# YifanXu74/MQ-Det

Hardware: NVIDIA H100
Metric: images/sec MQ-GLIP-T 800x1333, 5 vis-queries, 80-class prompt (higher is better)
Workload: dtype f16

## Files before the change

mqdet_b200/csrc/biattn.cu:

```cuda
#include "common.cuh"
#include "wgmma.cuh"
#include "../../include/mqdet_b200.h"

namespace mqdet {

constexpr int BM = 64;
constexpr int BK = 64;
constexpr int KB_BYTES = 64 * BK * 2;

template <int R>
__device__ __forceinline__ void acc_to_a(const float (&e)[R], int kk, uint32_t (&a)[4]) {
  a[0] = pack_half2(e[8 * kk + 0], e[8 * kk + 1]);
  a[1] = pack_half2(e[8 * kk + 2], e[8 * kk + 3]);
  a[2] = pack_half2(e[8 * kk + 4], e[8 * kk + 5]);
  a[3] = pack_half2(e[8 * kk + 6], e[8 * kk + 7]);
}
__device__ __forceinline__ float quad_max(float v) {
  v = fmaxf(v, __shfl_xor_sync(0xffffffffu, v, 1));
  return fmaxf(v, __shfl_xor_sync(0xffffffffu, v, 2));
}
__device__ __forceinline__ float quad_sum(float v) {
  v += __shfl_xor_sync(0xffffffffu, v, 1);
  return v + __shfl_xor_sync(0xffffffffu, v, 2);
}

constexpr int BT_STEP = 64;
struct BtCfg {
  static constexpr int KT_BYTES = 4 * KB_BYTES;
  static constexpr int Q_BYTES = 4 * KB_BYTES;
  static constexpr int V_BYTES = 256 * BT_STEP * 2;
  static constexpr int STAGE_BYTES = Q_BYTES + V_BYTES;
  static constexpr int SMEM_BYTES = KT_BYTES + 2 * STAGE_BYTES + 1024  + 256 ;
};
static_assert(BtCfg::SMEM_BYTES <= 232448, "biattn_text: dynamic shared memory above the 227 KB per-CTA limit");
struct BtP {
  const float* stat;
  float clamp;
  int nb1, T, N, n_steps;
  int k_bc1, k_bc2, q_bc1, q_bc2, v_bc1, v_bc2;
  const float* rowbias;
  int rb_ld;
  __half* out;
  long o_ld, o_b1, o_b2;
};

template <bool VN>
__global__ void __launch_bounds__(128, 1) biattn_text_kernel(const __grid_constant__ CUtensorMap tma_k,
                                                             const __grid_constant__ CUtensorMap tma_q,
                                                             const __grid_constant__ CUtensorMap tma_v, const BtP p) {
  extern __shared__ uint8_t smem_raw[];
  uint8_t* smem = reinterpret_cast<uint8_t*>((reinterpret_cast<uintptr_t>(smem_raw) + 1023) & ~uintptr_t(1023));
  uint8_t* kt = smem;
  uint8_t* ring = kt + BtCfg::KT_BYTES;
  uint64_t* bars = reinterpret_cast<uint64_t*>(ring + 2 * BtCfg::STAGE_BYTES);
  uint64_t* kt_full = bars;
  uint64_t* full = bars + 1;

  const int tid = threadIdx.x;
  const int mt = blockIdx.x, z = blockIdx.y;
  const int z1 = z % p.nb1, z2 = z / p.nb1;
  const int NS = p.n_steps;
  const int qz1 = p.q_bc1 ? 0 : z1, qz2 = p.q_bc2 ? 0 : z2, vz1 = p.v_bc1 ? 0 : z1, vz2 = p.v_bc2 ? 0 : z2;

  auto issue = [&](int i) {
    uint8_t* st = ring + (i & 1) * BtCfg::STAGE_BYTES;
    uint64_t* bar = &full[i & 1];
    mbar_expect_tx(bar, BtCfg::STAGE_BYTES);
    for (int kb = 0; kb < 4; ++kb) tma_load_4d(st + kb * KB_BYTES, &tma_q, bar, kb * BK, i * BT_STEP, qz1, qz2);
    if (VN)
      for (int cb = 0; cb < 4; ++cb) tma_load_4d(st + BtCfg::Q_BYTES + cb * KB_BYTES, &tma_v, bar, cb * BK, i * BT_STEP, vz1, vz2);
    else
      tma_load_4d(st + BtCfg::Q_BYTES, &tma_v, bar, i * BT_STEP, 0, vz1, vz2);
  };
  if (tid == 0) {
    tma_prefetch_desc(&tma_k);
    tma_prefetch_desc(&tma_q);
    tma_prefetch_desc(&tma_v);
    mbar_init(kt_full, 1);
    mbar_init(&full[0], 1);
    mbar_init(&full[1], 1);
    fence_mbar_init();
    mbar_expect_tx(kt_full, BtCfg::KT_BYTES);
    for (int kb = 0; kb < 4; ++kb)
      tma_load_4d(kt + kb * KB_BYTES, &tma_k, kt_full, kb * BK, mt * BM, p.k_bc1 ? 0 : z1, p.k_bc2 ? 0 : z2);
    issue(0);
    if (NS > 1) issue(1);
  }
  __syncthreads();

  constexpr float L2E = 1.4426950408889634f;
  float m_l2[2] = {0.f, 0.f}, inv[2] = {0.f, 0.f}, gb[2] = {0.f, 0.f}, lsum[2] = {0.f, 0.f};
#pragma unroll
  for (int h = 0; h < 2; ++h) {
    const int t = mt * BM + wg_row(tid, 2 * h);
    if (t < p.T) {
      if (VN) {
        m_l2[h] = -p.stat[(long)z * p.T + t] * L2E;
        if (p.rowbias) gb[h] = p.rowbias[((long)z * p.T + t) * p.rb_ld];
      } else {
        m_l2[h] = -p.stat[((long)z * 2) * p.T + t] * L2E;
        inv[h] = p.stat[((long)z * 2 + 1) * p.T + t];
      }
    }
  }
  const float clampv = p.clamp > 0.f ? p.clamp : 3.0e38f;
  const uint32_t kt_addr = smem_u32(kt);
  float o[128];
#pragma unroll
  for (int i = 0; i < 128; ++i) o[i] = 0.f;
  mbar_wait(kt_full, 0);
  for (int i = 0; i < NS; ++i) {
    const int s = i & 1;
    mbar_wait(&full[s], (i >> 1) & 1);
    const uint32_t q0 = smem_u32(ring + s * BtCfg::STAGE_BYTES), v0 = q0 + BtCfg::Q_BYTES;
    float sc[32];
#pragma unroll
    for (int j = 0; j < 32; ++j) sc[j] = 0.f;
    wgmma_fence_acc(sc);
    wgmma_fence();
#pragma unroll
    for (int kb = 0; kb < 4; ++kb)
#pragma unroll
      for (int k = 0; k < 4; ++k)
        wgmma_ss_m64n64_kk(sc, wg_desc_k_sw128(kt_addr + kb * KB_BYTES + k * 32), wg_desc_k_sw128(q0 + kb * KB_BYTES + k * 32), 1);
    wgmma_commit();
    wgmma_wait<0>();
    wgmma_fence_acc(sc);
    const int nrem = p.N - i * BT_STEP;
#pragma unroll
    for (int j = 0; j < 32; ++j) {
      const int h = (j >> 1) & 1;
      const float a = fminf(fmaxf(sc[j] + gb[h], -clampv), clampv);
      const float f = VN ? a : __half2float(__float2half_rn(a));
      float e = ex2_approx(fmaf(f, L2E, m_l2[h]));
      if (wg_col(tid, j) >= nrem) e = 0.f;
      if (VN) lsum[h] += e;
      sc[j] = e;
    }
    uint32_t pa[4][4];
#pragma unroll
    for (int kk = 0; kk < 4; ++kk) acc_to_a(sc, kk, pa[kk]);
    wgmma_fence_acc(o);
    wgmma_fence();
#pragma unroll
    for (int kk = 0; kk < 4; ++kk) {
      if (VN)
        wgmma_rs_m64n256_kmn(o, pa[kk], wg_desc_mn_sw128(v0 + kk * 2048, KB_BYTES, 1024), 1);
      else
        wgmma_rs_m64n256_kk(o, pa[kk], wg_desc_k_sw128(v0 + kk * 32), 1);
    }
    wgmma_commit();
    wgmma_wait<0>();
    wgmma_fence_acc(o);
    __syncthreads();
    if (tid == 0 && i + 2 < NS) issue(i + 2);
  }
  if (VN) {
#pragma unroll
    for (int h = 0; h < 2; ++h) {
      const float tot = quad_sum(lsum[h]);
      inv[h] = tot > 0.f ? 1.f / tot : 0.f;
    }
  }
  __half* out = p.out + z1 * p.o_b1 + z2 * p.o_b2;
#pragma unroll
  for (int j = 0; j < 128; j += 2) {
    const int h = (j >> 1) & 1;
    const int t = mt * BM + wg_row(tid, j);
    if (t < p.T)
      *reinterpret_cast<__half2*>(out + (long)t * p.o_ld + wg_col(tid, j)) = __floats2half2_rn(o[j] * inv[h], o[j + 1] * inv[h]);
  }
}

struct BiCfg {
  static constexpr int VN_BYTES = 4 * KB_BYTES;
  static constexpr int STAGE_BYTES = 256 * BK * 2;
  static constexpr int MAX_HEADS = 8;
  static constexpr int D_BYTES = 128 * 128 * 4;
  static constexpr int EXTRA_BYTES = (4 * 256 + MAX_HEADS * 256) * 4;
  static constexpr int SMEM_BYTES = VN_BYTES + 2 * STAGE_BYTES + D_BYTES + EXTRA_BYTES + 1024  + 256 ;
};
static_assert(BiCfg::SMEM_BYTES <= 232448, "biattn_image: dynamic shared memory above the 227 KB per-CTA limit");
struct BiP {
  const float* mask;
  const float* bias;
  const float* gamma;
  const __half* res;
  long res_ld, res_b;
  __half* out;
  long o_ld, o_b;
  float* colmax_part;
  const float* gbias;
  int gb_ld;
  float clamp;
  int B, H, T, N, tiles_per_img;
};

__global__ void __launch_bounds__(128, 1) biattn_image_kernel(const __grid_constant__ CUtensorMap tma_q,
                                                              const __grid_constant__ CUtensorMap tma_k,
                                                              const __grid_constant__ CUtensorMap tma_m, const BiP p) {
  extern __shared__ uint8_t smem_raw[];
  uint8_t* smem = reinterpret_cast<uint8_t*>((reinterpret_cast<uintptr_t>(smem_raw) + 1023) & ~uintptr_t(1023));
  uint8_t* vnt = smem;
  uint8_t* ring = vnt + BiCfg::VN_BYTES;
  float* dsum = reinterpret_cast<float*>(ring + 2 * BiCfg::STAGE_BYTES);
  float* cmx = dsum + 128 * 128;
  float* gk = cmx + 4 * 256;
  uint64_t* bars = reinterpret_cast<uint64_t*>(gk + BiCfg::MAX_HEADS * 256);
  uint64_t* vn_full = bars;
  uint64_t* full = bars + 1;

  const int tid = threadIdx.x, warp = tid >> 5, lane = tid & 31;
  const int H = p.H;
  const int b = blockIdx.x / p.tiles_per_img, ti = blockIdx.x - b * p.tiles_per_img, m0 = ti * BM;
  const int nq = 8 * H;
  auto issue = [&](int q) {
    const int h = q >> 3, kb = q & 3;
    uint64_t* bar = &full[q & 1];
    mbar_expect_tx(bar, BiCfg::STAGE_BYTES);
    tma_load_4d(ring + (q & 1) * BiCfg::STAGE_BYTES, (q & 4) ? &tma_m : &tma_k, bar, kb * BK, 0, h, b);
  };
  if (tid == 0) {
    tma_prefetch_desc(&tma_q);
    tma_prefetch_desc(&tma_k);
    tma_prefetch_desc(&tma_m);
    mbar_init(vn_full, 1);
    mbar_init(&full[0], 1);
    mbar_init(&full[1], 1);
    fence_mbar_init();
    mbar_expect_tx(vn_full, BiCfg::VN_BYTES);
    for (int kb = 0; kb < 4; ++kb) tma_load_4d(vnt + kb * KB_BYTES, &tma_q, vn_full, kb * BK, m0, b, 0);
    issue(0);
    issue(1);
  }
  constexpr float L2E = 1.4426950408889634f;
  const float NEG_INF = __int_as_float(0xff800000);
  const float clampv = p.clamp > 0.f ? p.clamp : 3.0e38f;
  for (int t = tid; t < 256; t += 128) {
    const bool kept = t < p.T && (!p.mask || p.mask[(long)b * p.T + t] != 0.f);
    for (int hh = 0; hh < H; ++hh)
      gk[hh * 256 + t] = !kept ? NEG_INF : (p.gbias ? p.gbias[(((long)b * H + hh) * p.T + t) * p.gb_ld] : 0.f);
  }
  __syncthreads();
  bool valid[2];
#pragma unroll
  for (int h = 0; h < 2; ++h) valid[h] = m0 + wg_row(tid, 2 * h) < p.N;
  const uint32_t vn_addr = smem_u32(vnt);
  int q = 0;
  auto ring_wait = [&](int qq) { mbar_wait(&full[qq & 1], (qq >> 1) & 1); };
  auto ring_release = [&](int qq) {
    __syncthreads();
    if (tid == 0 && qq + 2 < nq) issue(qq + 2);
  };
  mbar_wait(vn_full, 0);
  for (int h = 0; h < H; ++h) {
    float sc[128];
#pragma unroll
    for (int j = 0; j < 128; ++j) sc[j] = 0.f;
    for (int kb = 0; kb < 4; ++kb, ++q) {
      ring_wait(q);
      const uint32_t b0 = smem_u32(ring + (q & 1) * BiCfg::STAGE_BYTES);
      wgmma_fence_acc(sc);
      wgmma_fence();
#pragma unroll
      for (int k = 0; k < 4; ++k)
        wgmma_ss_m64n256_kk(sc, wg_desc_k_sw128(vn_addr + kb * KB_BYTES + k * 32), wg_desc_k_sw128(b0 + k * 32), 1);
      wgmma_commit();
      wgmma_wait<0>();
      wgmma_fence_acc(sc);
      ring_release(q);
    }
#pragma unroll
    for (int j = 0; j < 128; j += 4) {
#pragma unroll
      for (int c = 0; c < 2; ++c) {
        float m = fmaxf(valid[0] ? sc[j + c] : NEG_INF, valid[1] ? sc[j + 2 + c] : NEG_INF);
        m = fmaxf(m, __shfl_xor_sync(0xffffffffu, m, 4));
        m = fmaxf(m, __shfl_xor_sync(0xffffffffu, m, 8));
        m = fmaxf(m, __shfl_xor_sync(0xffffffffu, m, 16));
        if (lane < 4) cmx[warp * 256 + wg_col(tid, j + c)] = m;
      }
    }
    __syncthreads();
    for (int t = tid; t < p.T; t += 128) {
      float c4 = fmaxf(fmaxf(cmx[t], cmx[256 + t]), fmaxf(cmx[512 + t], cmx[768 + t]));
      if (p.gbias) c4 += p.gbias[(((long)b * H + h) * p.T + t) * p.gb_ld];
      c4 = fminf(fmaxf(c4, -clampv), clampv);
      p.colmax_part[(((long)b * H + h) * p.tiles_per_img + ti) * p.T + t] = c4;
    }
    const float* kl = gk + h * 256;
    float mr[2] = {NEG_INF, NEG_INF};
#pragma unroll
    for (int j = 0; j < 128; ++j) mr[(j >> 1) & 1] = fmaxf(mr[(j >> 1) & 1], sc[j] + kl[wg_col(tid, j)]);
    float ml2[2];
    bool uniform[2];
#pragma unroll
    for (int r = 0; r < 2; ++r) {
      const float m_raw = quad_max(mr[r]);
      uniform[r] = (m_raw == NEG_INF);
      ml2[r] = uniform[r] ? 0.f : fminf(fmaxf(m_raw, -clampv), clampv) * L2E;
    }
    float ls[2] = {0.f, 0.f};
#pragma unroll
    for (int j = 0; j < 128; ++j) {
      const int r = (j >> 1) & 1, c = wg_col(tid, j);
      const float kk = kl[c];
      float ev = (kk == NEG_INF) ? 0.f : ex2_approx(fmaf(fminf(fmaxf(sc[j] + kk, -clampv), clampv), L2E, -ml2[r]));
      if (uniform[r]) ev = (c < p.T) ? 1.f : 0.f;
      sc[j] = ev;
      ls[r] += ev;
    }
    const float inv[2] = {1.f / quad_sum(ls[0]), 1.f / quad_sum(ls[1])};
#pragma unroll
    for (int j = 0; j < 128; ++j) sc[j] *= inv[(j >> 1) & 1];
    uint32_t pa[16][4];
#pragma unroll
    for (int kk = 0; kk < 16; ++kk) acc_to_a(sc, kk, pa[kk]);
    float d[128];
#pragma unroll
    for (int j = 0; j < 128; ++j) d[j] = 0.f;
    for (int kb = 0; kb < 4; ++kb, ++q) {
      ring_wait(q);
      const uint32_t b0 = smem_u32(ring + (q & 1) * BiCfg::STAGE_BYTES);
      wgmma_fence_acc(d);
      wgmma_fence();
#pragma unroll
      for (int k = 0; k < 4; ++k) wgmma_rs_m64n256_kk(d, pa[kb * 4 + k], wg_desc_k_sw128(b0 + k * 32), 1);
      wgmma_commit();
      wgmma_wait<0>();
      wgmma_fence_acc(d);
      ring_release(q);
    }
#pragma unroll
    for (int j = 0; j < 128; ++j) dsum[j * 128 + tid] = (h == 0 ? 0.f : dsum[j * 128 + tid]) + d[j];
  }
#pragma unroll 4
  for (int j = 0; j < 128; j += 2) {
    const long row = m0 + wg_row(tid, j);
    const int c = wg_col(tid, j);
    if (row >= p.N) continue;
    float o0 = dsum[j * 128 + tid], o1 = dsum[(j + 1) * 128 + tid];
    const float g0 = p.gamma ? p.gamma[c] : 1.f, g1 = p.gamma ? p.gamma[c + 1] : 1.f;
    const float b0 = p.bias ? p.bias[c] : 0.f, b1 = p.bias ? p.bias[c + 1] : 0.f;
    o0 = (o0 + b0) * g0;
    o1 = (o1 + b1) * g1;
    if (p.res) {
      const float2 r = __half22float2(*reinterpret_cast<const __half2*>(p.res + (long)b * p.res_b + row * p.res_ld + c));
      o0 += r.x;
      o1 += r.y;
    }
    *reinterpret_cast<__half2*>(p.out + (long)b * p.o_b + row * p.o_ld + c) = __floats2half2_rn(o0, o1);
  }
}

__global__ void colmax_reduce_kernel(const float* __restrict__ part, int tiles, int T, float* __restrict__ out) {
  const int z = blockIdx.x;
  for (int t = threadIdx.x; t < T; t += blockDim.x) {
    float m = __int_as_float(0xff800000);
    const float* src = part + (long)z * tiles * T + t;
    for (int i = 0; i < tiles; ++i) m = fmaxf(m, src[(long)i * T]);
    out[(long)z * T + t] = m;
  }
}

}

using namespace mqdet;

static int text_launch(bool vn, const float* rowbias, int64_t rb_ld, const void* k, int64_t k_ld, int64_t k_b1, int64_t k_b2, const void* q, int64_t q_ld, int64_t q_b1,
                       int64_t q_b2, const void* v, int64_t v_ld, int64_t v_b1, int64_t v_b2, const float* stat, float clamp,
                       void* out, int64_t o_ld, int64_t o_b1, int64_t o_b2, int64_t nb1, int64_t nb2, int64_t T, int64_t N,
                       int64_t Np, int64_t d, void* stream) {
  MQ_REQUIRE(k && q && v && stat && out, "biattn_text: null pointer");
  MQ_REQUIRE(d == 256, "biattn_text: head dim must be 256 (embed 2048 / 8 heads, fuse_helper.py:186-189), got %ld", (long)d);
  MQ_REQUIRE(T >= 1 && T <= 256 && N >= 1 && Np >= N && (Np % 8) == 0, "biattn_text: need 1 <= T <= 256, Np >= N, Np %% 8 == 0");
  MQ_REQUIRE(nb1 >= 1 && nb2 >= 1 && nb1 * nb2 <= 65535, "biattn_text: bad batch");
  const int64_t lds[] = {k_ld, k_b1, k_b2, q_ld, q_b1, q_b2, v_ld, v_b1, v_b2, o_ld, o_b1, o_b2};
  for (int64_t x : lds) MQ_REQUIRE((x % 8) == 0, "biattn_text: strides must be multiples of 8 elements");
  MQ_REQUIRE(((uintptr_t)k % 16) == 0 && ((uintptr_t)q % 16) == 0 && ((uintptr_t)v % 16) == 0 && ((uintptr_t)out % 16) == 0,
             "biattn_text: operands must be 16-byte aligned");
  CUtensorMap mk, mq, mv;
  BtP p;
  memset(&p, 0, sizeof(p));
  int rc = make_operand_map(&mk, k, T, d, k_ld, (int)nb1, k_b1, (int)nb2, k_b2, BM, &p.k_bc1, &p.k_bc2);
  if (rc) return rc;
  rc = make_operand_map(&mq, q, N, d, q_ld, (int)nb1, q_b1, (int)nb2, q_b2, BT_STEP, &p.q_bc1, &p.q_bc2);
  if (rc) return rc;
  if (vn)
    rc = make_operand_map(&mv, v, N, 256, v_ld, (int)nb1, v_b1, (int)nb2, v_b2, BT_STEP, &p.v_bc1, &p.v_bc2);
  else
    rc = make_operand_map(&mv, v, d, Np, v_ld, (int)nb1, v_b1, (int)nb2, v_b2, 256, &p.v_bc1, &p.v_bc2);
  if (rc) return rc;
  MQ_REQUIRE((nb1 == 1 || o_b1 != 0) && (nb2 == 1 || o_b2 != 0), "biattn_text: output batch strides must be non-zero");
  p.out = (__half*)out;
  p.o_ld = o_ld;
  p.o_b1 = o_b1;
  p.o_b2 = o_b2;
  p.stat = stat;
  p.clamp = clamp;
  p.nb1 = (int)nb1;
  p.T = (int)T;
  p.N = (int)N;
  p.n_steps = (int)((N + BT_STEP - 1) / BT_STEP);
  p.rowbias = rowbias;
  p.rb_ld = (int)(rb_ld > 0 ? rb_ld : 1);
  dim3 grid((unsigned)((T + BM - 1) / BM), (unsigned)(nb1 * nb2));
  if (vn) {
    rc = ensure_dyn_smem(reinterpret_cast<const void*>(&biattn_text_kernel<true>), BtCfg::SMEM_BYTES);
    if (rc) return rc;
    biattn_text_kernel<true><<<grid, 128, BtCfg::SMEM_BYTES, (cudaStream_t)stream>>>(mk, mq, mv, p);
  } else {
    rc = ensure_dyn_smem(reinterpret_cast<const void*>(&biattn_text_kernel<false>), BtCfg::SMEM_BYTES);
    if (rc) return rc;
    biattn_text_kernel<false><<<grid, 128, BtCfg::SMEM_BYTES, (cudaStream_t)stream>>>(mk, mq, mv, p);
  }
  return check_launch("biattn_text_kernel");
}

extern "C" int mqdet_biattn_text(const void* k, int64_t k_ld, int64_t k_b1, int64_t k_b2, const void* q, int64_t q_ld,
                                 int64_t q_b1, int64_t q_b2, const void* vvT, int64_t v_ld, int64_t v_b1, int64_t v_b2,
                                 const float* stat, float clamp, void* out, int64_t o_ld, int64_t o_b1, int64_t o_b2,
                                 int64_t nb1, int64_t nb2, int64_t T, int64_t N, int64_t Np, int64_t d, void* stream) {
  return text_launch(false, nullptr, 0, k, k_ld, k_b1, k_b2, q, q_ld, q_b1, q_b2, vvT, v_ld, v_b1, v_b2, stat, clamp, out, o_ld, o_b1, o_b2,
                     nb1, nb2, T, N, Np, d, stream);
}

extern "C" int mqdet_biattn_text_vn(const void* k, int64_t k_ld, int64_t k_b1, int64_t k_b2, const void* q, int64_t q_ld,
                                    int64_t q_b1, int64_t q_b2, const void* vn, int64_t vn_ld, int64_t vn_b1, int64_t vn_b2,
                                    const float* colmax, const float* rowbias, int64_t rb_ld, float clamp, void* out, int64_t o_ld,
                                    int64_t o_b1, int64_t o_b2, int64_t nb1, int64_t nb2, int64_t T, int64_t N, void* stream) {
  return text_launch(true, rowbias, rb_ld, k, k_ld, k_b1, k_b2, q, q_ld, q_b1, q_b2, vn, vn_ld, vn_b1, vn_b2, colmax, clamp, out, o_ld, o_b1,
                     o_b2, nb1, nb2, T, N, (N + 7) / 8 * 8, 256, stream);
}

extern "C" int64_t mqdet_biattn_image_workspace_floats(int64_t B, int64_t H, int64_t N, int64_t T) {
  return B * H * ((N + BM - 1) / BM) * T;
}

extern "C" int mqdet_biattn_image(const void* vn, int64_t vn_ld, int64_t vn_b, const void* gT, int64_t g_ld, int64_t g_bh,
                                  int64_t g_b, const float* gbias, int64_t gb_ld, const void* mT, int64_t m_ld, int64_t m_bh,
                                  int64_t m_b, const float* bias, const float* gamma, const void* res, int64_t res_ld,
                                  int64_t res_b, const float* mask, float clamp, void* out, int64_t o_ld, int64_t o_b,
                                  float* colmax, float* workspace, int64_t B, int64_t H, int64_t N, int64_t T, void* stream) {
  MQ_REQUIRE(vn && gT && mT && out && colmax && workspace, "biattn_image: null pointer");
  MQ_REQUIRE(B >= 1 && H >= 1 && H <= BiCfg::MAX_HEADS && N >= 1 && T >= 8 && T <= 256 && (T % 8) == 0,
             "biattn_image: need B, N >= 1, 1 <= H <= 8, 8 <= T <= 256, T %% 8 == 0 (got B=%ld H=%ld N=%ld T=%ld)", (long)B, (long)H, (long)N, (long)T);
  const int64_t lds[] = {vn_ld, vn_b, g_ld, g_bh, g_b, m_ld, m_bh, m_b, o_ld, o_b, res ? res_ld : 0, res ? res_b : 0};
  for (int64_t x : lds) MQ_REQUIRE((x % 8) == 0, "biattn_image: strides must be multiples of 8 elements");
  MQ_REQUIRE(((uintptr_t)vn % 16) == 0 && ((uintptr_t)gT % 16) == 0 && ((uintptr_t)mT % 16) == 0 && ((uintptr_t)out % 16) == 0 &&
                 ((uintptr_t)res % 16) == 0 && ((uintptr_t)bias % 16) == 0 && ((uintptr_t)gamma % 16) == 0,
             "biattn_image: operands must be 16-byte aligned");
  CUtensorMap mq, mk, mm;
  int bc1, bc2;
  int rc = make_operand_map(&mq, vn, N, 256, vn_ld, (int)B, vn_b, 1, 0, BM, &bc1, &bc2);
  if (rc) return rc;
  MQ_REQUIRE((H == 1 || (g_bh != 0 && m_bh != 0)) && (B == 1 || (g_b != 0 && m_b != 0)), "biattn_image: head / image strides must be non-zero");
  rc = make_operand_map(&mk, gT, T, 256, g_ld, (int)H, g_bh, (int)B, g_b, 256, &bc1, &bc2);
  if (rc) return rc;
  rc = make_operand_map(&mm, mT, 256, T, m_ld, (int)H, m_bh, (int)B, m_b, 256, &bc1, &bc2);
  if (rc) return rc;
  MQ_REQUIRE(B == 1 || o_b != 0, "biattn_image: output batch stride must be non-zero");
  BiP p;
  memset(&p, 0, sizeof(p));
  p.mask = mask;
  p.bias = bias;
  p.gamma = gamma;
  p.res = (const __half*)res;
  p.res_ld = res_ld;
  p.res_b = res_b;
  p.out = (__half*)out;
  p.o_ld = o_ld;
  p.o_b = o_b;
  p.colmax_part = workspace;
  p.gbias = gbias;
  p.gb_ld = (int)(gb_ld > 0 ? gb_ld : 1);
  p.clamp = clamp;
  p.B = (int)B; p.H = (int)H; p.T = (int)T; p.N = (int)N;
  p.tiles_per_img = (int)((N + BM - 1) / BM);
  rc = ensure_dyn_smem(reinterpret_cast<const void*>(&biattn_image_kernel), BiCfg::SMEM_BYTES);
  if (rc) return rc;
  biattn_image_kernel<<<(unsigned)(p.tiles_per_img * B), 128, BiCfg::SMEM_BYTES, (cudaStream_t)stream>>>(mq, mk, mm, p);
  rc = check_launch("biattn_image_kernel");
  if (rc) return rc;
  colmax_reduce_kernel<<<(unsigned)(B * H), 256, 0, (cudaStream_t)stream>>>(workspace, p.tiles_per_img, (int)T, colmax);
  return check_launch("colmax_reduce_kernel");
}
```

mqdet_b200/csrc/common.cuh:

```cuda
#pragma once
#include <cuda.h>
#include <cuda_runtime.h>
#include <cuda_fp16.h>
#include <stdint.h>
#include <stdio.h>
#include <string.h>

#define MQDET_OK 0
#define MQDET_ERR_ARG -1
#define MQDET_ERR_CUDA -2
#define MQDET_ERR_UNSUPPORTED -3

namespace mqdet {

void set_error(const char* fmt, ...);
int check_launch(const char* what);

#define MQ_REQUIRE(cond, ...)                      \
  do {                                             \
    if (!(cond)) {                                 \
      mqdet::set_error(__VA_ARGS__);               \
      return MQDET_ERR_ARG;                        \
    }                                              \
  } while (0)
// ... 80 lines not shown
  d.pw = pw;
  d.ph = ph;
  return d;
}

__device__ __forceinline__ void token_focal_elem(float x, float y, float alpha, float gamma, float& loss, float& dloss) {
  const float p = 1.f / (1.f + expf(-x));
  const float ce = fmaxf(x, 0.f) - x * y + log1pf(expf(-fabsf(x)));
  const float pt = p * y + (1.f - p) * (1.f - y);
  const float om = 1.f - pt;
  const float mod = powf(om, gamma);
  const float at = alpha >= 0.f ? alpha * y + (1.f - alpha) * (1.f - y) : 1.f;
  loss = at * ce * mod;
  const float dmod = (om > 0.f) ? gamma * powf(om, gamma - 1.f) * (-(2.f * y - 1.f) * p * (1.f - p)) : 0.f;
  dloss = at * ((p - y) * mod + ce * dmod);
}

__device__ __forceinline__ void mbar_init(uint64_t* bar, uint32_t count) {
  asm volatile("mbarrier.init.shared::cta.b64 [%0], %1;" ::"r"(smem_u32(bar)), "r"(count));
}
__device__ __forceinline__ void fence_mbar_init() {
  asm volatile("fence.mbarrier_init.release.cluster;" ::: "memory");
}
__device__ __forceinline__ void sts128(uint32_t addr, uint32_t x, uint32_t y, uint32_t z, uint32_t w) {
  asm volatile("st.shared.v4.b32 [%0], {%1, %2, %3, %4};" ::"r"(addr), "r"(x), "r"(y), "r"(z), "r"(w) : "memory");
}
__device__ __forceinline__ float4 lds128f(uint32_t addr) {
  float4 v;
  asm volatile("ld.shared.v4.f32 {%0, %1, %2, %3}, [%4];" : "=f"(v.x), "=f"(v.y), "=f"(v.z), "=f"(v.w) : "r"(addr) : "memory");
  return v;
}
__device__ __forceinline__ float ex2_approx(float x) {
  float y;
  asm("ex2.approx.ftz.f32 %0, %1;" : "=f"(y) : "f"(x));
  return y;
}
__device__ __forceinline__ uint32_t pack_half2(float x, float y) {
  const __half2 h = __floats2half2_rn(x, y);
  return *reinterpret_cast<const uint32_t*>(&h);
}
__device__ __forceinline__ void ffma2(float& d0, float& d1, float a0, float a1, float s, float b0, float b1) {
  d0 = fmaf(a0, s, b0);
  d1 = fmaf(a1, s, b1);
}
__device__ __forceinline__ void ffma2v(float& d0, float& d1, float a0, float a1, float s0, float s1, float b0, float b1) {
  d0 = fmaf(a0, s0, b0);
  d1 = fmaf(a1, s1, b1);
}
__device__ __forceinline__ void fence_proxy_async() {
  asm volatile("fence.proxy.async.shared::cta;" ::: "memory");
}
__device__ __forceinline__ void mbar_expect_tx(uint64_t* bar, uint32_t bytes) {
  asm volatile("mbarrier.arrive.expect_tx.shared::cta.b64 _, [%0], %1;" ::"r"(smem_u32(bar)),
               "r"(bytes)
               : "memory");
}
__device__ __forceinline__ void mbar_arrive(uint64_t* bar) {
  asm volatile("mbarrier.arrive.shared::cta.b64 _, [%0];" ::"r"(smem_u32(bar)) : "memory");
}
__device__ __forceinline__ void mbar_wait(uint64_t* bar, uint32_t parity) {
  uint32_t addr = smem_u32(bar);
  uint32_t done;
  do {
    asm volatile(
        "{\n"
        ".reg .pred p;\n"
        "mbarrier.try_wait.parity.shared::cta.b64 p, [%1], %2;\n"
        "selp.u32 %0, 1, 0, p;\n"
        "}\n"
        : "=r"(done)
        : "r"(addr), "r"(parity)
        : "memory");
  } while (!done);
}

__device__ __forceinline__ void tma_prefetch_desc(const CUtensorMap* m) {
  asm volatile("prefetch.tensormap [%0];" ::"l"(reinterpret_cast<uint64_t>(m)) : "memory");
}
__device__ __forceinline__ void tma_load_4d(void* smem_dst, const CUtensorMap* m, uint64_t* bar,
                                            int c0, int c1, int c2, int c3) {
  asm volatile(
      "cp.async.bulk.tensor.4d.shared::cluster.global.tile.mbarrier::complete_tx::bytes "
// ... 83 lines not shown
```

mqdet_b200/csrc/gemm.cu:

```cuda
#include "common.cuh"
#include "wgmma.cuh"
#include "../../include/mqdet_b200.h"

namespace mqdet {

struct GemmP {
  const __half* A;
  const __half* B;
  long M, N, K, lda, ldb;
  int nb1, nb2;
  long a_b1, a_b2, b_b1, b_b2;
  void* C;
  int c_dtype;
  long ldc, c_b1, c_b2;
  float alpha;
  int scale_after_bias;
  const float* bias;
  int bias_mode;
  long bias_b1, bias_b2;
  int act;
  float clamp;
  const float* gate;
  int gate_mode, gate_tanh;
  const void* R;
// ... 56 lines not shown
  EPI_NONE_F16,
  EPI_BIAS_F16,
  EPI_BIAS_GELU_F16,
  EPI_BIAS_RES_F32,
};

template <int BN, int STAGES, int EPI>
struct WgCfg {
  static constexpr int A_BYTES = BM * BK * 2;
  static constexpr int B_BYTES = BN * BK * 2;
  static constexpr int STAGE_BYTES = A_BYTES + B_BYTES;
  static constexpr int PITCH = BN + 8;
  static constexpr bool OUT_F32 = EPI == EPI_BIAS_RES_F32;
  static constexpr int ES = OUT_F32 ? 4 : 2;
  static constexpr int PASSES = OUT_F32 ? 2 : 1;
  static constexpr int PASS_COLS = BN / PASSES;
  static constexpr int BOX_COLS = 128 / ES;
  static constexpr int BOXES = PASS_COLS / BOX_COLS;
  static constexpr int EPI_BYTES = EPI == EPI_GENERIC ? 64 * PITCH * 4 : BM * BN * 2;
  static constexpr int SMEM_BYTES = STAGES * STAGE_BYTES + 2 * EPI_BYTES + 1024  + 256 ;
  static_assert(EPI_BYTES % 1024 == 0, "swizzled boxes need 1024-byte alignment");
};

__device__ __forceinline__ void named_bar_sync(int id, int n) { asm volatile("bar.sync %0, %1;" ::"r"(id), "r"(n) : "memory"); }
__device__ __forceinline__ void named_bar_arrive(int id, int n) { asm volatile("bar.arrive %0, %1;" ::"r"(id), "r"(n) : "memory"); }
template <int R>
__device__ __forceinline__ void setmaxnreg_dec() { asm volatile("setmaxnreg.dec.sync.aligned.u32 %0;" ::"n"(R)); }
template <int R>
__device__ __forceinline__ void setmaxnreg_inc() { asm volatile("setmaxnreg.inc.sync.aligned.u32 %0;" ::"n"(R)); }
__device__ __forceinline__ void sts32(uint32_t addr, uint32_t x) { asm volatile("st.shared.b32 [%0], %1;" ::"r"(addr), "r"(x) : "memory"); }
__device__ __forceinline__ void sts64f(uint32_t addr, float x, float y) {
  asm volatile("st.shared.v2.f32 [%0], {%1, %2};" ::"r"(addr), "f"(x), "f"(y) : "memory");
}
__device__ __forceinline__ float2 lds64f(uint32_t addr) {
  float2 v;
  asm volatile("ld.shared.v2.f32 {%0, %1}, [%2];" : "=f"(v.x), "=f"(v.y) : "r"(addr) : "memory");
  return v;
}
template <int ES>
__device__ __forceinline__ uint32_t box_addr(uint32_t base, int r, int c) {
  const int byte = c * ES;
  return base + (byte >> 7) * (BM * 128) + r * 128 + ((((byte >> 4) & 7) ^ (r & 7)) << 4) + (byte & 15);
}

struct TileIdx {
  int n_tile, m_tile, z1, z2;
};
__device__ __forceinline__ TileIdx tile_idx(int t, int n_tiles, int m_tiles, int nb1) {
  TileIdx r;
  const int per_z = n_tiles * m_tiles;
  const int z = t / per_z, rem = t - z * per_z;
  r.m_tile = rem / n_tiles;
  r.n_tile = rem - r.m_tile * n_tiles;
// ... 396 lines not shown
```

Measured before the change: 178.6.

## Warp-specialize bi-attention kernels with producer warpgroup and split score/value consumers

Both bi-attention kernels become warp-specialized. One producer warpgroup drives TMA through full/empty mbarrier rings, and consumer warpgroups rebalance registers with setmaxnreg. The text kernel processes two M-tiles per CTA that share the streamed Q/V ring, and it reuses a single buffer when Q and V alias. The image kernel splits softmax scoring and the P·V product across two warpgroups that hand off probabilities through swizzled shared memory, with part of the accumulator spilled to shared memory. The column-max reduction is also parallelized across 8 warps. This aims to overlap loads, softmax and matmul and to cut full-CTA syncs, at the cost of more complex synchronization and fewer CTAs for the text kernel.

```diff
diff --git a/mqdet_b200/csrc/biattn.cu b/mqdet_b200/csrc/biattn.cu
--- a/mqdet_b200/csrc/biattn.cu
+++ b/mqdet_b200/csrc/biattn.cu
@@ -29,14 +29,16 @@
   static constexpr int KT_BYTES = 4 * KB_BYTES;
   static constexpr int Q_BYTES = 4 * KB_BYTES;
   static constexpr int V_BYTES = 256 * BT_STEP * 2;
-  static constexpr int STAGE_BYTES = Q_BYTES + V_BYTES;
-  static constexpr int SMEM_BYTES = KT_BYTES + 2 * STAGE_BYTES + 1024  + 256 ;
+  static constexpr int RING_BYTES = 2 * (Q_BYTES + V_BYTES);
+  static constexpr int MAX_STAGES = RING_BYTES / Q_BYTES;
+  static constexpr int SMEM_BYTES = 2 * KT_BYTES + RING_BYTES + 1024  + 256 ;
 };
 static_assert(BtCfg::SMEM_BYTES <= 232448, "biattn_text: dynamic shared memory above the 227 KB per-CTA limit");
 struct BtP {
   const float* stat;
   float clamp;
   int nb1, T, N, n_steps;
+  int qv_shared;
   int k_bc1, k_bc2, q_bc1, q_bc2, v_bc1, v_bc2;
   const float* rowbias;
   int rb_ld;
@@ -45,48 +47,72 @@
 };
 
 template <bool VN>
-__global__ void __launch_bounds__(128, 1) biattn_text_kernel(const __grid_constant__ CUtensorMap tma_k,
+__global__ void __launch_bounds__(384, 1) biattn_text_kernel(const __grid_constant__ CUtensorMap tma_k,
                                                              const __grid_constant__ CUtensorMap tma_q,
                                                              const __grid_constant__ CUtensorMap tma_v, const BtP p) {
   extern __shared__ uint8_t smem_raw[];
   uint8_t* smem = reinterpret_cast<uint8_t*>((reinterpret_cast<uintptr_t>(smem_raw) + 1023) & ~uintptr_t(1023));
   uint8_t* kt = smem;
-  uint8_t* ring = kt + BtCfg::KT_BYTES;
-  uint64_t* bars = reinterpret_cast<uint64_t*>(ring + 2 * BtCfg::STAGE_BYTES);
+  uint8_t* ring = kt + 2 * BtCfg::KT_BYTES;
+  uint64_t* bars = reinterpret_cast<uint64_t*>(ring + BtCfg::RING_BYTES);
   uint64_t* kt_full = bars;
-  uint64_t* full = bars + 1;
-
-  const int tid = threadIdx.x;
-  const int mt = blockIdx.x, z = blockIdx.y;
+  uint64_t* full = bars + 2;
+  uint64_t* empty = full + BtCfg::MAX_STAGES;
+
+  const int wg = threadIdx.x >> 7, tid = threadIdx.x & 127;
+  const int z = blockIdx.y;
   const int z1 = z % p.nb1, z2 = z / p.nb1;
   const int NS = p.n_steps;
-  const int qz1 = p.q_bc1 ? 0 : z1, qz2 = p.q_bc2 ? 0 : z2, vz1 = p.v_bc1 ? 0 : z1, vz2 = p.v_bc2 ? 0 : z2;
-
-  auto issue = [&](int i) {
-    uint8_t* st = ring + (i & 1) * BtCfg::STAGE_BYTES;
-    uint64_t* bar = &full[i & 1];
-    mbar_expect_tx(bar, BtCfg::STAGE_BYTES);
-    for (int kb = 0; kb < 4; ++kb) tma_load_4d(st + kb * KB_BYTES, &tma_q, bar, kb * BK, i * BT_STEP, qz1, qz2);
-    if (VN)
-      for (int cb = 0; cb < 4; ++cb) tma_load_4d(st + BtCfg::Q_BYTES + cb * KB_BYTES, &tma_v, bar, cb * BK, i * BT_STEP, vz1, vz2);
-    else
-      tma_load_4d(st + BtCfg::Q_BYTES, &tma_v, bar, i * BT_STEP, 0, vz1, vz2);
-  };
-  if (tid == 0) {
+  const int mt0 = 2 * blockIdx.x;
+  const int ncons = min(2, (p.T - mt0 * BM + BM - 1) / BM);
+  const int stage_bytes = p.qv_shared ? BtCfg::Q_BYTES : BtCfg::Q_BYTES + BtCfg::V_BYTES;
+  const int nst = BtCfg::RING_BYTES / stage_bytes;
+
+  if (threadIdx.x == 0) {
     tma_prefetch_desc(&tma_k);
     tma_prefetch_desc(&tma_q);
     tma_prefetch_desc(&tma_v);
-    mbar_init(kt_full, 1);
-    mbar_init(&full[0], 1);
-    mbar_init(&full[1], 1);
+    mbar_init(&kt_full[0], 1);
+    mbar_init(&kt_full[1], 1);
+    for (int s = 0; s < nst; ++s) {
+      mbar_init(&full[s], 1);
+      mbar_init(&empty[s], 128 * ncons);
+    }
     fence_mbar_init();
-    mbar_expect_tx(kt_full, BtCfg::KT_BYTES);
-    for (int kb = 0; kb < 4; ++kb)
-      tma_load_4d(kt + kb * KB_BYTES, &tma_k, kt_full, kb * BK, mt * BM, p.k_bc1 ? 0 : z1, p.k_bc2 ? 0 : z2);
-    issue(0);
-    if (NS > 1) issue(1);
   }
   __syncthreads();
+
+  if (wg == 0) {
+    setmaxnreg_dec<40>();
+    if (tid == 0) {
+      const int qz1 = p.q_bc1 ? 0 : z1, qz2 = p.q_bc2 ? 0 : z2, vz1 = p.v_bc1 ? 0 : z1, vz2 = p.v_bc2 ? 0 : z2;
+      for (int g = 0; g < ncons; ++g) {
+        mbar_expect_tx(&kt_full[g], BtCfg::KT_BYTES);
+        for (int kb = 0; kb < 4; ++kb)
+          tma_load_4d(kt + g * BtCfg::KT_BYTES + kb * KB_BYTES, &tma_k, &kt_full[g], kb * BK, (mt0 + g) * BM, p.k_bc1 ? 0 : z1,
+                      p.k_bc2 ? 0 : z2);
+      }
+      for (int i = 0; i < NS; ++i) {
+        const int s = i % nst;
+        uint8_t* st = ring + s * stage_bytes;
+        mbar_wait(&empty[s], ((i / nst) & 1) ^ 1);
+        mbar_expect_tx(&full[s], stage_bytes);
+        for (int kb = 0; kb < 4; ++kb) tma_load_4d(st + kb * KB_BYTES, &tma_q, &full[s], kb * BK, i * BT_STEP, qz1, qz2);
+        if (!p.qv_shared) {
+          if (VN)
+            for (int cb = 0; cb < 4; ++cb)
+              tma_load_4d(st + BtCfg::Q_BYTES + cb * KB_BYTES, &tma_v, &full[s], cb * BK, i * BT_STEP, vz1, vz2);
+          else
+            tma_load_4d(st + BtCfg::Q_BYTES, &tma_v, &full[s], i * BT_STEP, 0, vz1, vz2);
+        }
+      }
+    }
+    return;
+  }
+  setmaxnreg_inc<232>();
+  const int g = wg - 1;
+  if (g >= ncons) return;
+  const int mt = mt0 + g;
 
   constexpr float L2E = 1.4426950408889634f;
   float m_l2[2] = {0.f, 0.f}, inv[2] = {0.f, 0.f}, gb[2] = {0.f, 0.f}, lsum[2] = {0.f, 0.f};
@@ -104,15 +130,16 @@
     }
   }
   const float clampv = p.clamp > 0.f ? p.clamp : 3.0e38f;
-  const uint32_t kt_addr = smem_u32(kt);
+  const uint32_t kt_addr = smem_u32(kt + g * BtCfg::KT_BYTES);
+  const uint32_t v_off = p.qv_shared ? 0 : BtCfg::Q_BYTES;
   float o[128];
 #pragma unroll
   for (int i = 0; i < 128; ++i) o[i] = 0.f;
-  mbar_wait(kt_full, 0);
+  mbar_wait(&kt_full[g], 0);
   for (int i = 0; i < NS; ++i) {
-    const int s = i & 1;
-    mbar_wait(&full[s], (i >> 1) & 1);
-    const uint32_t q0 = smem_u32(ring + s * BtCfg::STAGE_BYTES), v0 = q0 + BtCfg::Q_BYTES;
+    const int s = i % nst;
+    mbar_wait(&full[s], (i / nst) & 1);
+    const uint32_t q0 = smem_u32(ring + s * stage_bytes), v0 = q0 + v_off;
     float sc[32];
 #pragma unroll
     for (int j = 0; j < 32; ++j) sc[j] = 0.f;
@@ -152,8 +179,7 @@
     wgmma_commit();
     wgmma_wait<0>();
     wgmma_fence_acc(o);
-    __syncthreads();
-    if (tid == 0 && i + 2 < NS) issue(i + 2);
+    mbar_arrive(&empty[s]);
   }
   if (VN) {
 #pragma unroll
@@ -175,10 +201,16 @@
 struct BiCfg {
   static constexpr int VN_BYTES = 4 * KB_BYTES;
   static constexpr int STAGE_BYTES = 256 * BK * 2;
+  static constexpr int STAGES = 2;
+  static constexpr int M_STAGE_BYTES = 64 * BK * 2;
+  static constexpr int M_STAGES = 4;
+  static constexpr int P_BYTES = 4 * KB_BYTES;
   static constexpr int MAX_HEADS = 8;
-  static constexpr int D_BYTES = 128 * 128 * 4;
-  static constexpr int EXTRA_BYTES = (4 * 256 + MAX_HEADS * 256) * 4;
-  static constexpr int SMEM_BYTES = VN_BYTES + 2 * STAGE_BYTES + D_BYTES + EXTRA_BYTES + 1024  + 256 ;
+  static constexpr int EXTRA_BYTES = (2 * 4 * 256 + MAX_HEADS * 256) * 4;
+  static constexpr int D_REG = 64;
+  static constexpr int D3_BYTES = (128 - D_REG) * 128 * 4;
+  static constexpr int SMEM_BYTES =
+      VN_BYTES + P_BYTES + STAGES * STAGE_BYTES + M_STAGES * M_STAGE_BYTES + EXTRA_BYTES + D3_BYTES + 1024  + 256 ;
 };
 static_assert(BiCfg::SMEM_BYTES <= 232448, "biattn_image: dynamic shared memory above the 227 KB per-CTA limit");
 struct BiP {
@@ -196,150 +228,209 @@
   int B, H, T, N, tiles_per_img;
 };
 
-__global__ void __launch_bounds__(128, 1) biattn_image_kernel(const __grid_constant__ CUtensorMap tma_q,
+__device__ __forceinline__ uint32_t sw128_off(int r, int c) {
+  return (c >> 6) * KB_BYTES + r * 128 + ((((c & 63) >> 3) ^ (r & 7)) << 4) + ((c & 7) << 1);
+}
+
+__global__ void __launch_bounds__(384, 1) biattn_image_kernel(const __grid_constant__ CUtensorMap tma_q,
                                                               const __grid_constant__ CUtensorMap tma_k,
                                                               const __grid_constant__ CUtensorMap tma_m, const BiP p) {
+  constexpr int S = BiCfg::STAGES, MS = BiCfg::M_STAGES;
   extern __shared__ uint8_t smem_raw[];
   uint8_t* smem = reinterpret_cast<uint8_t*>((reinterpret_cast<uintptr_t>(smem_raw) + 1023) & ~uintptr_t(1023));
   uint8_t* vnt = smem;
-  uint8_t* ring = vnt + BiCfg::VN_BYTES;
-  float* dsum = reinterpret_cast<float*>(ring + 2 * BiCfg::STAGE_BYTES);
-  float* cmx = dsum + 128 * 128;
-  float* gk = cmx + 4 * 256;
-  uint64_t* bars = reinterpret_cast<uint64_t*>(gk + BiCfg::MAX_HEADS * 256);
+  uint8_t* pt = vnt + BiCfg::VN_BYTES;
+  uint8_t* ring_g = pt + BiCfg::P_BYTES;
+  uint8_t* ring_m = ring_g + S * BiCfg::STAGE_BYTES;
+  float* cmx = reinterpret_cast<float*>(ring_m + MS * BiCfg::M_STAGE_BYTES);
+  float* gk = cmx + 2 * 4 * 256;
+  float* d3 = gk + BiCfg::MAX_HEADS * 256;
+  uint64_t* bars = reinterpret_cast<uint64_t*>(d3 + (128 - BiCfg::D_REG) * 128);
   uint64_t* vn_full = bars;
-  uint64_t* full = bars + 1;
-
-  const int tid = threadIdx.x, warp = tid >> 5, lane = tid & 31;
+  uint64_t* g_full = bars + 1;
+  uint64_t* g_empty = g_full + S;
+  uint64_t* m_full = g_empty + S;
+  uint64_t* m_empty = m_full + MS;
+  uint64_t* p_full = m_empty + MS;
+  uint64_t* p_empty = p_full + 1;
+
+  const int wg = threadIdx.x >> 7, tid = threadIdx.x & 127;
   const int H = p.H;
   const int b = blockIdx.x / p.tiles_per_img, ti = blockIdx.x - b * p.tiles_per_img, m0 = ti * BM;
-  const int nq = 8 * H;
-  auto issue = [&](int q) {
-    const int h = q >> 3, kb = q & 3;
-    uint64_t* bar = &full[q & 1];
-    mbar_expect_tx(bar, BiCfg::STAGE_BYTES);
-    tma_load_4d(ring + (q & 1) * BiCfg::STAGE_BYTES, (q & 4) ? &tma_m : &tma_k, bar, kb * BK, 0, h, b);
-  };
-  if (tid == 0) {
+  if (threadIdx.x == 0) {
     tma_prefetch_desc(&tma_q);
     tma_prefetch_desc(&tma_k);
     tma_prefetch_desc(&tma_m);
     mbar_init(vn_full, 1);
-    mbar_init(&full[0], 1);
-    mbar_init(&full[1], 1);
+    for (int s = 0; s < S; ++s) {
+      mbar_init(&g_full[s], 1);
+      mbar_init(&g_empty[s], 128);
+    }
+    for (int s = 0; s < MS; ++s) {
+      mbar_init(&m_full[s], 1);
+      mbar_init(&m_empty[s], 128);
+    }
+    mbar_init(p_full, 128);
+    mbar_init(p_empty, 128);
     fence_mbar_init();
-    mbar_expect_tx(vn_full, BiCfg::VN_BYTES);
-    for (int kb = 0; kb < 4; ++kb) tma_load_4d(vnt + kb * KB_BYTES, &tma_q, vn_full, kb * BK, m0, b, 0);
-    issue(0);
-    issue(1);
   }
   constexpr float L2E = 1.4426950408889634f;
   const float NEG_INF = __int_as_float(0xff800000);
   const float clampv = p.clamp > 0.f ? p.clamp : 3.0e38f;
-  for (int t = tid; t < 256; t += 128) {
+  for (int t = threadIdx.x; t < 256; t += 384) {
     const bool kept = t < p.T && (!p.mask || p.mask[(long)b * p.T + t] != 0.f);
     for (int hh = 0; hh < H; ++hh)
       gk[hh * 256 + t] = !kept ? NEG_INF : (p.gbias ? p.gbias[(((long)b * H + hh) * p.T + t) * p.gb_ld] : 0.f);
   }
   __syncthreads();
-  bool valid[2];
-#pragma unroll
-  for (int h = 0; h < 2; ++h) valid[h] = m0 + wg_row(tid, 2 * h) < p.N;
-  const uint32_t vn_addr = smem_u32(vnt);
+
+  if (wg == 0) {
+    setmaxnreg_dec<40>();
+    if (tid == 0) {
+      mbar_expect_tx(vn_full, BiCfg::VN_BYTES);
+      for (int kb = 0; kb < 4; ++kb) tma_load_4d(vnt + kb * KB_BYTES, &tma_q, vn_full, kb * BK, m0, b, 0);
+      for (int q = 0; q < 4 * H; ++q) {
+        const int s = q % S;
+        mbar_wait(&g_empty[s], ((q / S) & 1) ^ 1);
+        mbar_expect_tx(&g_full[s], BiCfg::STAGE_BYTES);
+        tma_load_4d(ring_g + s * BiCfg::STAGE_BYTES, &tma_k, &g_full[s], (q & 3) * BK, 0, q >> 2, b);
+      }
+    } else if (tid == 32) {
+      for (int q = 0; q < 16 * H; ++q) {
+        const int s = q % MS;
+        mbar_wait(&m_empty[s], ((q / MS) & 1) ^ 1);
+        mbar_expect_tx(&m_full[s], BiCfg::M_STAGE_BYTES);
+        tma_load_4d(ring_m + s * BiCfg::M_STAGE_BYTES, &tma_m, &m_full[s], (q & 3) * BK, ((q >> 2) & 3) * 64, q >> 4, b);
+      }
+    }
+    return;
+  }
+  setmaxnreg_inc<232>();
+
+  if (wg == 1) {
+    const int warp = tid >> 5, lane = tid & 31;
+    bool valid[2];
+#pragma unroll
+    for (int h = 0; h < 2; ++h) valid[h] = m0 + wg_row(tid, 2 * h) < p.N;
+    const uint32_t vn_addr = smem_u32(vnt), p_addr = smem_u32(pt);
+    mbar_wait(vn_full, 0);
+    int q = 0;
+    for (int h = 0; h < H; ++h) {
+      float sc[128];
+#pragma unroll
+      for (int j = 0; j < 128; ++j) sc[j] = 0.f;
+      for (int kb = 0; kb < 4; ++kb, ++q) {
+        const int s = q % S;
+        mbar_wait(&g_full[s], (q / S) & 1);
+        const uint32_t b0 = smem_u32(ring_g + s * BiCfg::STAGE_BYTES);
+        wgmma_fence_acc(sc);
+        wgmma_fence();
+#pragma unroll
+        for (int k = 0; k < 4; ++k)
+          wgmma_ss_m64n256_kk(sc, wg_desc_k_sw128(vn_addr + kb * KB_BYTES + k * 32), wg_desc_k_sw128(b0 + k * 32), 1);
+        wgmma_commit();
+        wgmma_wait<0>();
+        wgmma_fence_acc(sc);
+        mbar_arrive(&g_empty[s]);
+      }
+      float* cm = cmx + (h & 1) * 4 * 256;
+#pragma unroll
+      for (int j = 0; j < 128; j += 4) {
+#pragma unroll
+        for (int c = 0; c < 2; ++c) {
+          float m = fmaxf(valid[0] ? sc[j + c] : NEG_INF, valid[1] ? sc[j + 2 + c] : NEG_INF);
+          m = fmaxf(m, __shfl_xor_sync(0xffffffffu, m, 4));
+          m = fmaxf(m, __shfl_xor_sync(0xffffffffu, m, 8));
+          m = fmaxf(m, __shfl_xor_sync(0xffffffffu, m, 16));
+          if (lane < 4) cm[warp * 256 + wg_col(tid, j + c)] = m;
+        }
+      }
+      named_bar_sync(1, 128);
+      for (int t = tid; t < p.T; t += 128) {
+        float c4 = fmaxf(fmaxf(cm[t], cm[256 + t]), fmaxf(cm[512 + t], cm[768 + t]));
+        if (p.gbias) c4 += p.gbias[(((long)b * H + h) * p.T + t) * p.gb_ld];
+        c4 = fminf(fmaxf(c4, -clampv), clampv);
+        p.colmax_part[(((long)b * H + h) * p.tiles_per_img + ti) * p.T + t] = c4;
+      }
+      const float* kl = gk + h * 256;
+      float mr[2] = {NEG_INF, NEG_INF};
+#pragma unroll
+      for (int j = 0; j < 128; ++j) mr[(j >> 1) & 1] = fmaxf(mr[(j >> 1) & 1], sc[j] + kl[wg_col(tid, j)]);
+      float ml2[2];
+      bool uniform[2];
+#pragma unroll
+      for (int r = 0; r < 2; ++r) {
+        const float m_raw = quad_max(mr[r]);
+        uniform[r] = (m_raw == NEG_INF);
+        ml2[r] = uniform[r] ? 0.f : fminf(fmaxf(m_raw, -clampv), clampv) * L2E;
+      }
+      float ls[2] = {0.f, 0.f};
+#pragma unroll
+      for (int j = 0; j < 128; ++j) {
+        const int r = (j >> 1) & 1, c = wg_col(tid, j);
+        const float kk = kl[c];
+        float ev = (kk == NEG_INF) ? 0.f : ex2_approx(fmaf(fminf(fmaxf(sc[j] + kk, -clampv), clampv), L2E, -ml2[r]));
+        if (uniform[r]) ev = (c < p.T) ? 1.f : 0.f;
+        sc[j] = ev;
+        ls[r] += ev;
+      }
+      const float inv[2] = {1.f / quad_sum(ls[0]), 1.f / quad_sum(ls[1])};
+      if (h > 0) mbar_wait(p_empty, (h - 1) & 1);
+#pragma unroll
+      for (int j = 0; j < 128; j += 2) {
+        const int r = (j >> 1) & 1;
+        sts32(p_addr + sw128_off(wg_row(tid, j), wg_col(tid, j)), pack_half2(sc[j] * inv[r], sc[j + 1] * inv[r]));
+      }
+      fence_proxy_async();
+      mbar_arrive(p_full);
+    }
+    return;
+  }
+
+  constexpr int DR = BiCfg::D_REG;
+  const uint32_t p_addr = smem_u32(pt);
+  float d[DR];
+#pragma unroll
+  for (int j = 0; j < DR; ++j) d[j] = 0.f;
   int q = 0;
-  auto ring_wait = [&](int qq) { mbar_wait(&full[qq & 1], (qq >> 1) & 1); };
-  auto ring_release = [&](int qq) {
-    __syncthreads();
-    if (tid == 0 && qq + 2 < nq) issue(qq + 2);
-  };
-  mbar_wait(vn_full, 0);
   for (int h = 0; h < H; ++h) {
-    float sc[128];
-#pragma unroll
-    for (int j = 0; j < 128; ++j) sc[j] = 0.f;
-    for (int kb = 0; kb < 4; ++kb, ++q) {
-      ring_wait(q);
-      const uint32_t b0 = smem_u32(ring + (q & 1) * BiCfg::STAGE_BYTES);
-      wgmma_fence_acc(sc);
-      wgmma_fence();
-#pragma unroll
-      for (int k = 0; k < 4; ++k)
-        wgmma_ss_m64n256_kk(sc, wg_desc_k_sw128(vn_addr + kb * KB_BYTES + k * 32), wg_desc_k_sw128(b0 + k * 32), 1);
-      wgmma_commit();
-      wgmma_wait<0>();
-      wgmma_fence_acc(sc);
-      ring_release(q);
-    }
-#pragma unroll
-    for (int j = 0; j < 128; j += 4) {
-#pragma unroll
-      for (int c = 0; c < 2; ++c) {
-        float m = fmaxf(valid[0] ? sc[j + c] : NEG_INF, valid[1] ? sc[j + 2 + c] : NEG_INF);
-        m = fmaxf(m, __shfl_xor_sync(0xffffffffu, m, 4));
-        m = fmaxf(m, __shfl_xor_sync(0xffffffffu, m, 8));
-        m = fmaxf(m, __shfl_xor_sync(0xffffffffu, m, 16));
-        if (lane < 4) cmx[warp * 256 + wg_col(tid, j + c)] = m;
-      }
-    }
-    __syncthreads();
-    for (int t = tid; t < p.T; t += 128) {
-      float c4 = fmaxf(fmaxf(cmx[t], cmx[256 + t]), fmaxf(cmx[512 + t], cmx[768 + t]));
-      if (p.gbias) c4 += p.gbias[(((long)b * H + h) * p.T + t) * p.gb_ld];
-      c4 = fminf(fmaxf(c4, -clampv), clampv);
-      p.colmax_part[(((long)b * H + h) * p.tiles_per_img + ti) * p.T + t] = c4;
-    }
-    const float* kl = gk + h * 256;
-    float mr[2] = {NEG_INF, NEG_INF};
-#pragma unroll
-    for (int j = 0; j < 128; ++j) mr[(j >> 1) & 1] = fmaxf(mr[(j >> 1) & 1], sc[j] + kl[wg_col(tid, j)]);
-    float ml2[2];
-    bool uniform[2];
-#pragma unroll
-    for (int r = 0; r < 2; ++r) {
-      const float m_raw = quad_max(mr[r]);
-      uniform[r] = (m_raw == NEG_INF);
-      ml2[r] = uniform[r] ? 0.f : fminf(fmaxf(m_raw, -clampv), clampv) * L2E;
-    }
-    float ls[2] = {0.f, 0.f};
-#pragma unroll
-    for (int j = 0; j < 128; ++j) {
-      const int r = (j >> 1) & 1, c = wg_col(tid, j);
-      const float kk = kl[c];
-      float ev = (kk == NEG_INF) ? 0.f : ex2_approx(fmaf(fminf(fmaxf(sc[j] + kk, -clampv), clampv), L2E, -ml2[r]));
-      if (uniform[r]) ev = (c < p.T) ? 1.f : 0.f;
-      sc[j] = ev;
-      ls[r] += ev;
-    }
-    const float inv[2] = {1.f / quad_sum(ls[0]), 1.f / quad_sum(ls[1])};
-#pragma unroll
-    for (int j = 0; j < 128; ++j) sc[j] *= inv[(j >> 1) & 1];
-    uint32_t pa[16][4];
-#pragma unroll
-    for (int kk = 0; kk < 16; ++kk) acc_to_a(sc, kk, pa[kk]);
-    float d[128];
-#pragma unroll
-    for (int j = 0; j < 128; ++j) d[j] = 0.f;
-    for (int kb = 0; kb < 4; ++kb, ++q) {
-      ring_wait(q);
-      const uint32_t b0 = smem_u32(ring + (q & 1) * BiCfg::STAGE_BYTES);
-      wgmma_fence_acc(d);
-      wgmma_fence();
-#pragma unroll
-      for (int k = 0; k < 4; ++k) wgmma_rs_m64n256_kk(d, pa[kb * 4 + k], wg_desc_k_sw128(b0 + k * 32), 1);
-      wgmma_commit();
-      wgmma_wait<0>();
-      wgmma_fence_acc(d);
-      ring_release(q);
-    }
-#pragma unroll
-    for (int j = 0; j < 128; ++j) dsum[j * 128 + tid] = (h == 0 ? 0.f : dsum[j * 128 + tid]) + d[j];
-  }
-#pragma unroll 4
+    mbar_wait(p_full, h & 1);
+#pragma unroll
+    for (int qc = 0; qc < 4; ++qc) {
+      float dh[32];
+#pragma unroll
+      for (int j = 0; j < 32; ++j) dh[j] = 0.f;
+      for (int kb = 0; kb < 4; ++kb, ++q) {
+        const int s = q % MS;
+        mbar_wait(&m_full[s], (q / MS) & 1);
+        const uint32_t b0 = smem_u32(ring_m + s * BiCfg::M_STAGE_BYTES);
+        wgmma_fence_acc(dh);
+        wgmma_fence();
+#pragma unroll
+        for (int k = 0; k < 4; ++k)
+          wgmma_ss_m64n64_kk(dh, wg_desc_k_sw128(p_addr + kb * KB_BYTES + k * 32), wg_desc_k_sw128(b0 + k * 32), 1);
+        wgmma_commit();
+        wgmma_wait<0>();
+        wgmma_fence_acc(dh);
+        mbar_arrive(&m_empty[s]);
+      }
+#pragma unroll
+      for (int j = 0; j < 32; ++j) {
+        const int i = qc * 32 + j;
+        if (i < DR)
+          d[i] += dh[j];
+        else
+          d3[(i - DR) * 128 + tid] = (h == 0 ? 0.f : d3[(i - DR) * 128 + tid]) + dh[j];
+      }
+    }
+    mbar_arrive(p_empty);
+  }
+#pragma unroll
   for (int j = 0; j < 128; j += 2) {
     const long row = m0 + wg_row(tid, j);
     const int c = wg_col(tid, j);
     if (row >= p.N) continue;
-    float o0 = dsum[j * 128 + tid], o1 = dsum[(j + 1) * 128 + tid];
+    float o0 = j < DR ? d[j] : d3[(j - DR) * 128 + tid], o1 = j < DR ? d[j + 1] : d3[(j + 1 - DR) * 128 + tid];
     const float g0 = p.gamma ? p.gamma[c] : 1.f, g1 = p.gamma ? p.gamma[c + 1] : 1.f;
     const float b0 = p.bias ? p.bias[c] : 0.f, b1 = p.bias ? p.bias[c + 1] : 0.f;
     o0 = (o0 + b0) * g0;
@@ -353,12 +444,19 @@
   }
 }
 
-__global__ void colmax_reduce_kernel(const float* __restrict__ part, int tiles, int T, float* __restrict__ out) {
-  const int z = blockIdx.x;
-  for (int t = threadIdx.x; t < T; t += blockDim.x) {
-    float m = __int_as_float(0xff800000);
+__global__ void __launch_bounds__(256) colmax_reduce_kernel(const float* __restrict__ part, int tiles, int T, float* __restrict__ out) {
+  __shared__ float red[8][32];
+  const int z = blockIdx.x, t = blockIdx.y * 32 + threadIdx.x, w = threadIdx.y;
+  float m = __int_as_float(0xff800000);
+  if (t < T) {
     const float* src = part + (long)z * tiles * T + t;
-    for (int i = 0; i < tiles; ++i) m = fmaxf(m, src[(long)i * T]);
+    for (int i = w; i < tiles; i += 8) m = fmaxf(m, src[(long)i * T]);
+  }
+  red[w][threadIdx.x] = m;
+  __syncthreads();
+  if (w == 0 && t < T) {
+#pragma unroll
+    for (int k = 1; k < 8; ++k) m = fmaxf(m, red[k][threadIdx.x]);
     out[(long)z * T + t] = m;
   }
 }
@@ -404,15 +502,17 @@
   p.n_steps = (int)((N + BT_STEP - 1) / BT_STEP);
   p.rowbias = rowbias;
   p.rb_ld = (int)(rb_ld > 0 ? rb_ld : 1);
-  dim3 grid((unsigned)((T + BM - 1) / BM), (unsigned)(nb1 * nb2));
+  p.qv_shared = vn && q == v && q_ld == v_ld && p.q_bc1 == p.v_bc1 && p.q_bc2 == p.v_bc2 && (p.q_bc1 || q_b1 == v_b1) &&
+                (p.q_bc2 || q_b2 == v_b2);
+  dim3 grid((unsigned)((T + 2 * BM - 1) / (2 * BM)), (unsigned)(nb1 * nb2));
   if (vn) {
     rc = ensure_dyn_smem(reinterpret_cast<const void*>(&biattn_text_kernel<true>), BtCfg::SMEM_BYTES);
     if (rc) return rc;
-    biattn_text_kernel<true><<<grid, 128, BtCfg::SMEM_BYTES, (cudaStream_t)stream>>>(mk, mq, mv, p);
+    biattn_text_kernel<true><<<grid, 384, BtCfg::SMEM_BYTES, (cudaStream_t)stream>>>(mk, mq, mv, p);
   } else {
     rc = ensure_dyn_smem(reinterpret_cast<const void*>(&biattn_text_kernel<false>), BtCfg::SMEM_BYTES);
     if (rc) return rc;
-    biattn_text_kernel<false><<<grid, 128, BtCfg::SMEM_BYTES, (cudaStream_t)stream>>>(mk, mq, mv, p);
+    biattn_text_kernel<false><<<grid, 384, BtCfg::SMEM_BYTES, (cudaStream_t)stream>>>(mk, mq, mv, p);
   }
   return check_launch("biattn_text_kernel");
 }
@@ -457,7 +557,7 @@
   MQ_REQUIRE((H == 1 || (g_bh != 0 && m_bh != 0)) && (B == 1 || (g_b != 0 && m_b != 0)), "biattn_image: head / image strides must be non-zero");
   rc = make_operand_map(&mk, gT, T, 256, g_ld, (int)H, g_bh, (int)B, g_b, 256, &bc1, &bc2);
   if (rc) return rc;
-  rc = make_operand_map(&mm, mT, 256, T, m_ld, (int)H, m_bh, (int)B, m_b, 256, &bc1, &bc2);
+  rc = make_operand_map(&mm, mT, 256, T, m_ld, (int)H, m_bh, (int)B, m_b, 64, &bc1, &bc2);
   if (rc) return rc;
   MQ_REQUIRE(B == 1 || o_b != 0, "biattn_image: output batch stride must be non-zero");
   BiP p;
@@ -479,9 +579,10 @@
   p.tiles_per_img = (int)((N + BM - 1) / BM);
   rc = ensure_dyn_smem(reinterpret_cast<const void*>(&biattn_image_kernel), BiCfg::SMEM_BYTES);
   if (rc) return rc;
-  biattn_image_kernel<<<(unsigned)(p.tiles_per_img * B), 128, BiCfg::SMEM_BYTES, (cudaStream_t)stream>>>(mq, mk, mm, p);
+  biattn_image_kernel<<<(unsigned)(p.tiles_per_img * B), 384, BiCfg::SMEM_BYTES, (cudaStream_t)stream>>>(mq, mk, mm, p);
   rc = check_launch("biattn_image_kernel");
   if (rc) return rc;
-  colmax_reduce_kernel<<<(unsigned)(B * H), 256, 0, (cudaStream_t)stream>>>(workspace, p.tiles_per_img, (int)T, colmax);
+  colmax_reduce_kernel<<<dim3((unsigned)(B * H), (unsigned)((T + 31) / 32)), dim3(32, 8), 0, (cudaStream_t)stream>>>(
+      workspace, p.tiles_per_img, (int)T, colmax);
   return check_launch("colmax_reduce_kernel");
 }
diff --git a/mqdet_b200/csrc/common.cuh b/mqdet_b200/csrc/common.cuh
--- a/mqdet_b200/csrc/common.cuh
+++ b/mqdet_b200/csrc/common.cuh
@@ -126,6 +126,7 @@
 __device__ __forceinline__ void fence_mbar_init() {
   asm volatile("fence.mbarrier_init.release.cluster;" ::: "memory");
 }
+__device__ __forceinline__ void sts32(uint32_t addr, uint32_t x) { asm volatile("st.shared.b32 [%0], %1;" ::"r"(addr), "r"(x) : "memory"); }
 __device__ __forceinline__ void sts128(uint32_t addr, uint32_t x, uint32_t y, uint32_t z, uint32_t w) {
   asm volatile("st.shared.v4.b32 [%0], {%1, %2, %3, %4};" ::"r"(addr), "r"(x), "r"(y), "r"(z), "r"(w) : "memory");
 }
@@ -162,6 +163,13 @@
 __device__ __forceinline__ void mbar_arrive(uint64_t* bar) {
   asm volatile("mbarrier.arrive.shared::cta.b64 _, [%0];" ::"r"(smem_u32(bar)) : "memory");
 }
+__device__ __forceinline__ void named_bar_sync(int id, int n) { asm volatile("bar.sync %0, %1;" ::"r"(id), "r"(n) : "memory"); }
+__device__ __forceinline__ void named_bar_arrive(int id, int n) { asm volatile("bar.arrive %0, %1;" ::"r"(id), "r"(n) : "memory"); }
+template <int R>
+__device__ __forceinline__ void setmaxnreg_dec() { asm volatile("setmaxnreg.dec.sync.aligned.u32 %0;" ::"n"(R)); }
+template <int R>
+__device__ __forceinline__ void setmaxnreg_inc() { asm volatile("setmaxnreg.inc.sync.aligned.u32 %0;" ::"n"(R)); }
+
 __device__ __forceinline__ void mbar_wait(uint64_t* bar, uint32_t parity) {
   uint32_t addr = smem_u32(bar);
   uint32_t done;
diff --git a/mqdet_b200/csrc/gemm.cu b/mqdet_b200/csrc/gemm.cu
--- a/mqdet_b200/csrc/gemm.cu
+++ b/mqdet_b200/csrc/gemm.cu
@@ -102,13 +102,6 @@
   static_assert(EPI_BYTES % 1024 == 0, "swizzled boxes need 1024-byte alignment");
 };
 
-__device__ __forceinline__ void named_bar_sync(int id, int n) { asm volatile("bar.sync %0, %1;" ::"r"(id), "r"(n) : "memory"); }
-__device__ __forceinline__ void named_bar_arrive(int id, int n) { asm volatile("bar.arrive %0, %1;" ::"r"(id), "r"(n) : "memory"); }
-template <int R>
-__device__ __forceinline__ void setmaxnreg_dec() { asm volatile("setmaxnreg.dec.sync.aligned.u32 %0;" ::"n"(R)); }
-template <int R>
-__device__ __forceinline__ void setmaxnreg_inc() { asm volatile("setmaxnreg.inc.sync.aligned.u32 %0;" ::"n"(R)); }
-__device__ __forceinline__ void sts32(uint32_t addr, uint32_t x) { asm volatile("st.shared.b32 [%0], %1;" ::"r"(addr), "r"(x) : "memory"); }
 __device__ __forceinline__ void sts64f(uint32_t addr, float x, float y) {
   asm volatile("st.shared.v2.f32 [%0], {%1, %2};" ::"r"(addr), "f"(x), "f"(y) : "memory");
 }
```

Measured after the change: 184.5 (median of 6 runs). +3.3%, better.
